# JacobYuan7/DIN-Group-Activity-Recognition-Benchmark

Hardware: AMD Instinct MI355X
Metric: clips/sec (fwd+bwd), Volleyball DIN stage-2, BxTx12 actors (higher is better)
Workload: dtype bf16; 1 GPU; Volleyball stage-2 DIN, inv3, T=3, ST_kernel=(3,3), N=12, 720x1280, bf16; global_batch=32, clips_per_gpu=32, frames=3, parallelism=dp1, includes=fwd + cross-entropy + bwd + fused Adam (lr 0), launch_mode=eager launches, bn_mode=running statistics (set_bn_eval)

## Files before the change

### din-group-activity-recognition-benchmark_amd/_lib.py

```python
from __future__ import annotations

import ctypes as C
import os
import re
import subprocess
from typing import Dict, List

_HERE = os.path.dirname(os.path.abspath(__file__))
LIB_PATH = os.environ.get("DIN_LIB_PATH") or os.path.join(_HERE, "libdin_hip.so")
CSRC_DIR = os.path.join(_HERE, "csrc")
HEADER_PATH = os.path.join(os.path.dirname(_HERE), "include", "din_hip.h")

DIN_F32, DIN_BF16 = 0, 1
ABI_VERSION = 9
CONV_BIAS, CONV_RELU, CONV_ACCUM, CONV_MASK = 1, 2, 4, 8


class DinError(RuntimeError):
    pass


class ConvDesc(C.Structure):
    _fields_ = [(n, C.c_int32) for n in (
        "nb", "h", "w", "cin", "oh", "ow", "cout", "kh", "kw", "sh", "sw", "ph", "pw", "dh", "dw",
# ... 23 lines not shown
    _fields_ = [("desc", ConvDesc), ("in_", C.c_void_p), ("dout", C.c_void_p), ("dw", C.c_void_p), ("dbias", C.c_void_p), ("scale", C.c_void_p),
                ("w", C.c_void_p), ("wdot", C.c_void_p), ("accumulate", C.c_int32), ("reserved", C.c_int32)]


_P, _I, _L, _F, _U64 = C.c_void_p, C.c_int, C.c_int64, C.c_float, C.c_uint64
_CD, _PD = C.POINTER(ConvDesc), C.POINTER(PoolDesc)

SIGNATURES: Dict[str, tuple] = {
    "din_abi_version": (_I, []),
    "din_last_error_string": (C.c_char_p, []),
    "din_set_option": (_I, [C.c_char_p, C.c_char_p]),
    "din_get_option": (_I, [C.c_char_p, C.c_char_p, _I]),
    "din_build_arch": (C.c_char_p, []),
    "din_prep_images_f32": (_I, [_P, _P, _L, _P]),
    "din_prep_images_nhwc": (_I, [_P, _I, _P, _I, _I, _I, _I, _I, _P]),
    "din_conv_packed_elems": (_L, [_CD, _I]),
    "din_conv_pack_weights": (_I, [_CD, _P, _P, _P, _I, _P]),
    "din_conv_pack_desc": (_I, [_CD, _P, _P, _P, _I, C.POINTER(PackDesc)]),
    "din_conv_pack_multi": (_I, [_P, _P, _P, _I, _I, _P]),
    "din_conv_kernel_tile": (_I, [_CD, _I, C.POINTER(C.c_int32), C.POINTER(C.c_int32)]),
    "din_conv_kernel_variant": (_I, [_CD, _I, C.POINTER(C.c_int32)]),
    "din_conv_workspace_bytes": (_L, [_CD, _I]),
    "din_conv_accepts_u8": (_I, [_P]),
    "din_conv_fwd": (_I, [_CD, _P, _P, _P, _P, _I, _P, _L, _P]),
    "din_conv_fwd2": (_I, [_CD, _P, _P, _P, _P, _P, _I, _I, _I, _I, _I, _P, _L, _P]),
    "din_conv_dgrad": (_I, [_CD, _P, _P, _P, _P, _I, _I, _I, _P, _L, _P]),
    "din_conv1x1_dgrad_multi": (_I, [_I, C.POINTER(ConvSrc), _I, _I, _I, _I, _I, _I, _I, _P, _P, _I, _I, _I, _P]),
    "din_conv_dgrad_x_fused": (_I, [_CD]),
    "din_conv_dgrad_x": (_I, [_CD, _P, _P, _P, _P, _I, _I, _I, C.POINTER(ConvSrc), _P, _L, _P]),
    "din_conv1x1_wgrad_multi_workspace": (_L, [_I, C.POINTER(ConvWSrc), _I, _L, _I]),
    "din_conv1x1_wgrad_multi": (_I, [_I, C.POINTER(ConvWSrc), _I, _L, _I, _I, _I, _P, _I, _P, _L, _P]),
    "din_conv_wgrad_group_key": (_I, [_CD]),
    "din_conv_wgrad_group_workspace": (_L, [_I, C.POINTER(ConvWgradItem)]),
    "din_conv_wgrad_group": (_I, [_I, C.POINTER(ConvWgradItem), _P, _L, _P]),
    "din_conv_wgrad": (_I, [_CD, _P, _P, _P, _P, _P, _P, _P, _I, _P, _L, _P]),
    "din_colsum": (_I, [_P, _I, _L, _I, _I, _I, _P, _P]),
    "din_bn_fold": (_I, [_P, _P, _P, _P, _F, _P, _P, _I, _P]),
    "din_bn_fold_bwd": (_I, [_P, _P, _P, _P, _F, _P, _P, _I, _P]),
    "din_bn_fold_multi": (_I, [_P, _P, _I, _I, _F, _P, _P, _P]),
    "din_bn_fold_bwd_multi": (_I, [_P, _P, _I, _I, _F, _P, _P, _P, _P, _P]),
    "din_bn_stats": (_I, [_P, _I, _L, _I, _I, _I, _P, _P, _P]),
    "din_bn_parts": (_I, [_L]),
    "din_bn_workspace": (_L, [_L, _I]),
    "din_bn_reduce": (_I, [_P, _I, _I, _P]),
    "din_bn_finalize": (_I, [_P, _I, _L, _I, _P, _P, _F, _F, _P, _P, _P, _P, _P, _P, _P, _P]),
    "din_bn_apply": (_I, [_P, _I, _L, _I, _I, _I, _P, _P, _I, _P, _I, _I, _P]),
# ... 114 lines not shown
```

### din-group-activity-recognition-benchmark_amd/csrc/conv_igemm.hip

```cpp
#include "din_common.h"
#include "conv_wgrad.h"
#include "conv_gather.h"
#include <atomic>
#include <unordered_map>
#include <mutex>
#include <stdlib.h>

typedef float f32x4 __attribute__((ext_vector_type(4)));
typedef __bf16 bf16x8 __attribute__((ext_vector_type(8)));
typedef uint32_t u32x4 __attribute__((ext_vector_type(4)));
typedef uint32_t u32x2 __attribute__((ext_vector_type(2)));

using din_wgrad::WgradK;
using din_wgrad::lds_dma16;
using din_gather::ConvK;
using din_gather::out_pixel;
using din_gather::staged_tile_store;

namespace {

#ifndef DIN_GATHER_PRIO
#define DIN_GATHER_PRIO 0
#endif
#ifndef DIN_GATHER_ILV
#define DIN_GATHER_ILV 1
#endif
constexpr int BM = 128;
constexpr int KC = 8;
constexpr int NTHREADS = 256;

__device__ __forceinline__ int lds_slot(int row, int chunk) { return row * KC + (chunk ^ ((row >> 1) & 7)); }

template <typename T> struct Mma;
template <> struct Mma<float> {
    __device__ static void run(const u32x4& a, const u32x4& b, f32x4& c) {
#pragma unroll
        for (int j = 0; j < 4; ++j)
            c = __builtin_amdgcn_mfma_f32_16x16x4f32(__uint_as_float(a[j]), __uint_as_float(b[j]), c, 0, 0, 0);
    }
};
// ... 576 lines not shown
        const int px_l = wm * (BM / WM) + (lane & 15);
#pragma unroll
        for (int i = 0; i < TI; ++i) {
            f32x4 bv = {0.f, 0.f, 0.f, 0.f};
            const int co = co_tile * BN + co_l + i * 16;
            const bool cooked = p.craw <= 0 || co < p.craw;
            if ((p.flags & DIN_CONV_BIAS) && co < p.Cout && cooked) bv = *reinterpret_cast<const f32x4*>(p.bias + co);
#pragma unroll
            for (int j = 0; j < TJ; ++j) {
                f32x4 v = acc[i][j] + bv;
                if ((p.flags & DIN_CONV_RELU) && cooked) {
#pragma unroll
                    for (int e = 0; e < 4; ++e) v[e] = fmaxf(v[e], 0.f);
                }
                unsigned char* dst = smem_raw + (px_l + j * 16) * CPITCH + (co_l + i * 16) * (int)sizeof(T);
                if constexpr (sizeof(T) == 4) *reinterpret_cast<f32x4*>(dst) = v;
                else *reinterpret_cast<u32x2*>(dst) = u32x2{pack_bf16x2(v[0], v[1]), pack_bf16x2(v[2], v[3])};
            }
        }
    }
    staged_tile_store<T, BM, BN, NT>(p, smem_raw, tid, co_tile, m_first);
#endif
}

__device__ __forceinline__ float prep_u8(uint32_t v) {
    float y = __fdiv_rn((float)v, 255.0f);
    y = __fsub_rn(y, 0.5f);
    return __fmul_rn(y, 2.0f);
}
__device__ __forceinline__ void u8_lut_init(bf16_t* lut, int tid) {
    lut[tid] = (bf16_t)(pack_bf16x2(prep_u8((uint32_t)tid), 0.f) & 0xffffu);
}
template <int V> struct IcTag { static constexpr int value = V; };
template <int NTR>
struct U8Halo {
    uint32_t r[NTR], g[NTR], b[NTR];
    uint32_t valid;
    template <int NSLOT>
    __device__ __forceinline__ void load(const unsigned char* __restrict__ img, int n, int H, int W, int gy0, int gx0, int wid,
                                         const short (&hyv)[NTR], const short (&hxv)[NTR], const int (&inside)[NTR]) {
        const int64_t plane = (int64_t)H * W;
        const unsigned char* base = img + (int64_t)n * 3 * plane;
        valid = 0u;
#pragma unroll
        for (int i = 0; i < NTR; ++i) {
            const int gy = gy0 + hyv[i], gx = gx0 + hxv[i];
            const bool ok = wid + 4 * i < NSLOT && inside[i] >= 0 && gy >= 0 && gy < H && gx >= 0 && gx < W;
            const unsigned char* q = base + (int64_t)min(max(gy, 0), H - 1) * W + min(max(gx, 0), W - 1);
            asm volatile("global_load_ubyte %0, %1, off" : "=&v"(r[i]) : "v"(q) : "memory");
            asm volatile("global_load_ubyte %0, %1, off" : "=&v"(g[i]) : "v"(q + plane) : "memory");
            asm volatile("global_load_ubyte %0, %1, off" : "=&v"(b[i]) : "v"(q + 2 * plane) : "memory");
            valid |= (ok ? 1u : 0u) << i;
        }
    }
    __device__ __forceinline__ void landed() {
#pragma unroll
        for (int i = 0; i < NTR; ++i) { asm volatile("" : "+v"(r[i])); asm volatile("" : "+v"(g[i])); asm volatile("" : "+v"(b[i])); }
    }
    template <int NSLOT>
    __device__ __forceinline__ void store(unsigned char* lds_buf, const bf16_t* lut, int wid, int lane) const {
#pragma unroll
        for (int i = 0; i < NTR; ++i) {
            if (wid + 4 * i < NSLOT) {
                u32x4 v = {0u, 0u, 0u, 0u};
                if ((valid >> i) & 1u) {
                    v[0] = (uint32_t)lut[r[i]] | ((uint32_t)lut[g[i]] << 16);
                    v[1] = (uint32_t)lut[b[i]];
                }
                *reinterpret_cast<u32x4*>(lds_buf + ((wid + 4 * i) * 64 + lane) * 16) = v;
            }
        }
    }
};

template <int CPP, int BN, int NBUF, int KH, int KW, int ST, bool U8 = false, int NW = 4, bool EPI = false>
__global__ __launch_bounds__(64 * NW, NW == 8 ? 1 : 2) void conv_small_kernel(ConvK p) {
    constexpr int NTHREADS = 64 * NW;
    static_assert(!U8 || NW == 4, "the uint8 halo loader is written for four waves");
    static_assert(!U8 || (CPP == 1 && NBUF == 2), "uint8 frames feed the image layer only");
#if defined(__HIP_DEVICE_COMPILE__)
    typedef bf16_t T;
    constexpr int TH = 8, TW = 32, NPX = TH * TW;
    constexpr int TI = BN / 16, TJ = 16 / NW, NTAPS = KH * KW;
    constexpr int SL = CPP >= 4 ? CPP / 4 : 1, NSL = CPP >= 4 ? NTAPS * SL : (NTAPS + 3) / 4;
    constexpr int CPITCH = BN * 2 + 16;
    constexpr int HWW = (TW - 1) * ST + KW, HWH = (TH - 1) * ST + KH, HPX = HWW * HWH, HC = HPX * CPP;
    constexpr int WBYTES = NSL * BN * 4 * 16;
    constexpr int HBYTES = (HC * 16 + 1023) / 1024 * 1024;
    constexpr int NSLOT = HBYTES / 1024, NTR = (NSLOT + NW - 1) / NW;
    constexpr int NPASS = HBYTES / CPITCH >= NPX ? 1 : 2;
    static_assert(HBYTES / CPITCH >= NPX / NPASS, "staging does not fit the halo buffer");
    constexpr int JN = TJ / NPASS;
    constexpr int CPR = BN / 8;
    constexpr int NST = (NPX / NPASS) * CPR / NTHREADS * NPASS;
    static_assert((NPX / NPASS) * CPR % NTHREADS == 0, "store loop must be uniform");
    constexpr unsigned OOB = 0x80000000u;
// ... 2989 lines not shown
```

### din-group-activity-recognition-benchmark_amd/nhwc.py

```python
from __future__ import annotations

import ctypes as C
from dataclasses import dataclass, field
from typing import Dict, List, Optional, Sequence, Tuple

import torch

from . import _lib as L


def _ptr(t: Optional[torch.Tensor]):
    return C.c_void_p(t.data_ptr()) if t is not None else None


def _stream():
    return C.c_void_p(torch.cuda.current_stream().cuda_stream)


def torch_dtype(dt: int):
    return torch.float32 if dt == L.DIN_F32 else torch.bfloat16


def din_dtype(t: torch.Tensor) -> int:
    if t.dtype == torch.float32:
# ... 19 lines not shown


def _timed(kind, d, name=""):
    return LAUNCH_TIMER(kind, d, name) if LAUNCH_TIMER is not None else _contextlib.nullcontext()


GRAD_HOOK = None
GRAD_TAP = None
GRAD_BUFFER = None
GRAD_ASSIGN = None


def _dw_buffer(w: torch.Tensor) -> torch.Tensor:
    if GRAD_BUFFER is not None:
        buf = GRAD_BUFFER(w)
        if buf is not None:
            return buf
    return torch.empty_like(w)
FUSE_1X1_DGRAD = None
FUSE_FWD_SIBLINGS = None
FUSE_WGRAD_SIBLINGS = None
FUSE_WGRAD_1X1 = None
FUSE_DGRAD_X = None
GROUP_WGRAD = None
GROUP_WGRAD_MAX = 12
GROUP_WGRAD_MB = 768
_SWITCHES = {"FUSE_1X1_DGRAD": ("DIN_FUSE_1X1", True), "FUSE_FWD_SIBLINGS": ("DIN_FUSE_FWD", True), "FUSE_WGRAD_SIBLINGS": ("DIN_FUSE_WGRAD", True),
             "FUSE_WGRAD_1X1": ("DIN_FUSE_WGRAD_1X1", True), "FUSE_DGRAD_X": ("DIN_FUSE_DGRAD_X", True), "GROUP_WGRAD": ("DIN_GROUP_WGRAD", True), "WGRAD_SIDE_STREAM": ("DIN_WGRAD_STREAM", False)}


def switch(attr: str) -> bool:
    v = globals()[attr]
    if v is not None:
        return bool(v)
    name, default = _SWITCHES[attr]
    return L.host_flag(name, default)



_WS: Dict[Tuple[int, str], torch.Tensor] = {}


_SIDE: Dict[int, "torch.cuda.Stream"] = {}
WGRAD_SIDE_STREAM = None


def side_stream(device) -> "torch.cuda.Stream":
    key = device.index if device.index is not None else torch.cuda.current_device()
    if key not in _SIDE:
        _SIDE[key] = torch.cuda.Stream(device=device)
    return _SIDE[key]
# ... 270 lines not shown
            op = g.ops[oi]
            d = _conv_desc(g, op, 1, dt, op.src.c)
            w, scale_ptr = src_of[oi]
            pd = L.PackDesc()
            L.check(lib.din_conv_pack_desc(C.byref(d), _ptr(w), scale_ptr, _ptr(fused), 0, C.byref(pd)), "conv_pack_desc(fused)")
            pd.out = fused.data_ptr() + row0 * pd.kelems * esz
            pd.rows_pad = pd.rows
            li = len(descs)
            descs.append(pd)
            nchunk = (pd.rows * pd.kelems + PACK_CHUNK - 1) // PACK_CHUNK
            layer_of += [li] * nchunk
            chunk_index += list(range(nchunk))
            row0 += op.dst.c
    raw = (L.PackDesc * len(descs))(*descs)
    host = torch.frombuffer(bytearray(bytes(raw)), dtype=torch.uint8).clone()
    pc.table = host.to(dev)
    pc.layer_of = torch.tensor(layer_of, dtype=torch.int32).to(dev)
    pc.chunk_index = torch.tensor(chunk_index, dtype=torch.int32).to(dev)
    pc.nblocks = len(layer_of)
    g._pack_cache = pc
    return pc


BN_MOMENTUM = 0.1


def _bn_train_forward(lib, raw: torch.Tensor, dt: int, rows: int, cout: int, gamma, beta, mean, var, relu: bool, dst: torch.Tensor,
                      ldd: int, coffd: int, st):
    dev = raw.device
    ws = torch.empty(lib.din_bn_workspace(rows, cout) // 8, dtype=torch.float64, device=dev)
    ab = torch.empty(4 * cout, dtype=torch.float32, device=dev)
    a, b, bmean, rstd = ab[:cout], ab[cout:2 * cout], ab[2 * cout:3 * cout], ab[3 * cout:]
    L.check(lib.din_bn_stats(_ptr(raw), dt, rows, cout, cout, 0, None, _ptr(ws), st), "bn_stats")
    L.check(lib.din_bn_finalize(_ptr(ws), lib.din_bn_parts(rows), rows, cout, _ptr(gamma), _ptr(beta), BN_EPS, BN_MOMENTUM, _ptr(mean), _ptr(var),
                                _ptr(a), _ptr(b), _ptr(bmean), _ptr(rstd), None, st), "bn_finalize")
    L.check(lib.din_bn_apply(_ptr(raw), dt, rows, cout, cout, 0, _ptr(a), _ptr(b), int(relu), _ptr(dst), ldd, coffd, st), "bn_apply")
    return bmean, rstd


def graph_forward(g: Graph, image_buf: torch.Tensor, params: Sequence[torch.Tensor], dt: int, save_for_backward: bool = True,
                  bn_train: bool = False):
    lib = L.load()
    nb = image_buf.shape[0]
    dev = image_buf.device
    tdt = torch_dtype(dt)
    bufs: List[Optional[torch.Tensor]] = [None] * len(g.tensors)
    bufs[g.input_tid] = image_buf
    it = iter(params)
    aux = []
    st = _stream()
    bn = _bn_tables(g, params, dev)
    pc = _pack_cache(g, params, dt, dev, save_for_backward, bn)
    bn_train = bool(bn_train) and bn is not None
    if bn_train:
        bn_scale, bn_shift = pc.bn_scale, pc.bn_shift
        bn_scale.fill_(1.0)
    elif bn is not None:
        bn_scale, bn_shift = pc.bn_scale, pc.bn_shift
        L.check(lib.din_bn_fold_multi(_ptr(bn.ptrs), _ptr(bn.offs), bn.n, bn.total, BN_EPS, _ptr(bn_scale), _ptr(bn_shift), st), "bn_fold_multi")
    L.check(lib.din_conv_pack_multi(_ptr(pc.table), _ptr(pc.layer_of), _ptr(pc.chunk_index), pc.nblocks, PACK_CHUNK, st), "conv_pack_multi")
    bn_i = 0
    group_of = {grp[0]: grp for grp in g.fwd_groups} if (switch("FUSE_FWD_SIBLINGS") and not bn_train) else {}
    fused_done = set()
    for oi, op in enumerate(g.ops):
        td = g.tensors[op.dst.tid]
        if bufs[op.dst.tid] is None:
            bufs[op.dst.tid] = torch.empty((nb, td.h, td.w, td.c), dtype=tdt, device=dev)
        src, dst = bufs[op.src.tid], bufs[op.dst.tid]
        if op.kind == "conv":
            cin = g.cin_image if op.src.tid == g.input_tid else op.src.c
            d = _conv_desc(g, op, nb, dt, cin)
            if op.src.tid == g.input_tid and src.dtype == torch.uint8:
                d.in_u8, d.ldi, d.cioff = 1, 8, 0
            w = next(it)
            scale = shift = None
            if op.bn:
                gamma, beta, mean, var = next(it), next(it), next(it), next(it)
                o0, o1 = bn.off_list[bn_i], bn.off_list[bn_i + 1]
                bn_i += 1
                scale, shift = bn_scale[o0:o1], bn_shift[o0:o1]
                bias = shift
            else:
                bias = next(it) if op.bias else None
            if op.bn and bn_train:
                dR = _conv_desc(g, op, nb, dt, cin)
                dR.in_u8, dR.ldi, dR.cioff = d.in_u8, d.ldi, d.cioff
                dR.ldo, dR.cooff = op.dst.c, 0
                raw = torch.empty((nb, g.tensors[op.src.tid].h if op.pooled is not None else td.h,
                                   g.tensors[op.src.tid].w if op.pooled is not None else td.w, op.dst.c), dtype=tdt, device=dev)
                if op.pooled is not None:
                    dR.oh, dR.ow = raw.shape[1], raw.shape[2]
                ws, wsb = workspace(lib.din_conv_workspace_bytes(C.byref(dR), 0), dev)
                with _timed("fwd", dR, op.name):
                    L.check(lib.din_conv_fwd(C.byref(dR), _ptr(src), _ptr(pc.wpk[oi]), None, _ptr(raw), 0, _ptr(ws), wsb, st), "conv_fwd " + op.name)
                if op.pooled is not None:
                    _, pd = _pooled_descs(g, op, nb, dt)
                    pd.ldo, pd.cooff = op.dst.c, 0
                    pooled_raw = torch.empty((nb, td.h, td.w, op.dst.c), dtype=tdt, device=dev)
                    L.check(lib.din_avgpool_fwd(C.byref(pd), _ptr(raw), _ptr(pooled_raw), None, 0, st), "avgpool_fwd(raw)")
                    raw = pooled_raw
                bmean, rstd = _bn_train_forward(lib, raw, dt, nb * td.h * td.w, op.dst.c, gamma, beta, mean, var, op.relu, dst, td.c,
                                                op.dst.coff, st)
                aux.append((None, raw if save_for_backward else None, bmean, rstd))
                continue
            if oi in fused_done:
                if op.pooled is not None:
                    _, pd = _pooled_descs(g, op, nb, dt)
                    pd.ldi, pd.cioff = g.tensors[op.mid.tid].c, op.mid.coff
                    L.check(lib.din_avgpool_fwd(C.byref(pd), _ptr(bufs[op.mid.tid]), _ptr(dst), _ptr(bias),
                                                L.CONV_BIAS | (L.CONV_RELU if op.relu else 0), st), "avgpool_fwd(epilogue)")
                aux.append((scale,))
                continue
            if oi in group_of and op.bn:
                grp = group_of[oi]
                rest = [g.ops[i] for i in grp[1:]]
                ctot = op.dst.c + sum(o.dst.c for o in rest)
                craw = ctot - sum(o.dst.c for o in rest if o.pooled is not None)
                dF = _conv_desc(g, op, nb, dt, cin)
                dF.cout = ctot
                v2 = group_view(rest[0])
                t2 = v2.tid
                td2 = g.tensors[t2]
                if lib.din_conv_workspace_bytes(C.byref(dF), 0) == 0 and bn.off_list[bn_i - 1 + len(grp)] - o0 == ctot:
                    if bufs[t2] is None:
                        bufs[t2] = torch.empty((nb, td2.h, td2.w, td2.c), dtype=tdt, device=dev)
                    flags = L.CONV_BIAS | (L.CONV_RELU if op.relu else 0)
# ... 581 lines not shown
```

### din-group-activity-recognition-benchmark_amd/profiling.py

```python
from __future__ import annotations

import ctypes as C
import os

import torch

from . import _lib as L
from . import nhwc

PROFILE = None
PROFILE_ONLY = None
HBM = None


def _conv_flops(d) -> float:
    over = getattr(d, "flops_override", None)
    return float(over) if over else 2.0 * d.nb * d.oh * d.ow * d.cout * d.cin * d.kh * d.kw


def _esz(dt: int) -> int:
    return 4 if dt == L.DIN_F32 else 2


def _stem_bytes(kind: str, d) -> float:
    e = _esz(d.dtype)
    x = d.nb * d.h * d.w * (3 if d.in_u8 else d.cin * e)
    y = d.nb * d.oh * d.ow * d.cout * e
    if kind == "fwd":
        return float(x + y)
    if kind == "dgrad":
        return float(y + 2 * x)
    return float(x + y)


def _pool_bytes(name: str, args) -> float:
    d = args[0]._obj
    e = _esz(d.dtype)
    big, small = d.nb * d.h * d.w * d.c, d.nb * d.oh * d.ow * d.c
    if name == "din_maxpool_fwd":
        return float(e * (big + small) + (small if args[3] else 0))
    return float(e * (small + big) + (small if args[2] else e * big) + (e * big if args[6] else 0))


def _roi_bytes(name: str, args) -> float:
    if name == "din_roi_align_fwd":
        _fm, dt, nb, hf, wf, c, _ldf, _gh, _gw, _b, _i, m, k = args[:13]
        return float(nb * hf * wf * c * _esz(dt) + m * c * k * k * 4)
    if name == "din_roi_crop_grad_transpose":
# ... 47 lines not shown
            setattr(lib, name, fn)
        self.records, HBM = HBM, None
        return False

    def summary(self, event_overhead_ms: float = 0.0, peak_gbs: float = 8000.0):
        out = {}
        for group, _name, nbytes, e0, e1 in self.records:
            rec = out.setdefault(group, [0.0, 0.0, 0])
            rec[0] += nbytes
            rec[1] += max(e0.elapsed_time(e1) - event_overhead_ms, 1e-4) * 1e-3
            rec[2] += 1
        return {g: {"bound": "hbm", "achieved": round(v[0] / v[1] / 1e9, 1), "peak": peak_gbs, "unit": "GB/s",
                    "frac": round(v[0] / v[1] / 1e9 / peak_gbs, 4), "launches": v[2], "time_ms": round(v[1] * 1e3, 3),
                    "algorithmic_bytes": round(v[0])} for g, v in out.items()}


class LaunchTimer:
    def __init__(self, kind, d, name=""):
        self.kind, self.d, self.name = kind, d, name
        self.rec = False

    def _variant(self) -> str:
        d = self.d
        bm, bn = C.c_int32(0), C.c_int32(0)
        which = {"fwd": 0, "dgrad": 1, "wgrad": 2}[self.kind]
        L.load().din_conv_kernel_tile(C.byref(d), which, C.byref(bm), C.byref(bn))
        tn = "unsigned short" if d.dtype == L.DIN_BF16 else "float"
        if self.kind == "wgrad":
            if self.name.startswith("1x1multi:"):
                return f"conv_wgrad_1x1_multi_kernel<{d.cin // 8}>"
            if self.name.startswith("group:"):
                return f"conv_wgrad_pipe_group_kernel<{bm.value}, {bn.value - 2000}, {'true' if d.ow >= 32 else 'false'}, 8>"
            if bm.value == 3:
                return f"conv_wgrad_halo_kernel<..., {bn.value}, ...>"
            if bm.value == 0:
                return f"conv_wgrad_small_kernel<..., {bn.value}, ...>"
            if bn.value >= 2000:
                waves = int(L.get_option("DIN_WGRAD_PIPE_WAVES") or "16")
                wn = 8 if waves == 16 else (2 if waves == 4 and bm.value <= 192 else 4)
                return f"conv_wgrad_pipe_kernel<{bm.value}, {bn.value - 2000}, {'true' if d.ow >= 32 else 'false'}, {wn}>"
            if bn.value >= 1000:
                return f"conv_wgrad_ring_kernel<{bm.value}, {bn.value - 1000}>"
            return f"conv_wgrad_bf16_kernel<{bm.value}>" if d.dtype == L.DIN_BF16 else "conv_wgrad_f32_kernel"
        if bm.value == 4 and not (self.kind == "dgrad" and "+" in self.name):
            return f"conv1x1_stream_kernel<{bn.value}>"
        if bm.value == 5:
# ... 16 lines not shown
        if BM == 256:
            geo = "4, 1, 4, 4" if BN == 64 else ("2, 2, 8, 2" if BN in (96, 160) else "4, 2, 8, 2")
        elif multi:
            geo = "4, 2, 8, 2" if (BN % 64 == 0 and d.dtype == L.DIN_BF16) else "2, 2, 8, 2"
        else:
            geo = "4, 2, 8, 2" if fl.value & 2 else "2, 2, 8, 2"
        return (f"conv_gather_fast_kernel<{tn}, {BM}, {BN}, {geo}, {'true' if multi else 'false'}, "
                f"{'true' if fl.value & 1 else 'false'}, false, {'true' if fl.value & 4 else 'false'}>")

    def __enter__(self):
        if PROFILE is not None:
            self.variant = self._variant()
            if PROFILE_ONLY is None or self.variant == PROFILE_ONLY:
                self.rec = True
                self.e0 = torch.cuda.Event(enable_timing=True)
                self.e1 = torch.cuda.Event(enable_timing=True)
                self.e0.record(torch.cuda.current_stream())
        return self

    def __exit__(self, *exc):
        if self.rec:
            self.e1.record(torch.cuda.current_stream())
            PROFILE.append((self.kind, self.variant, _conv_flops(self.d), int(self.d.dtype), self.e0, self.e1, self.name))
            if HBM is not None and self.variant.startswith(("conv_small_kernel", "conv_wgrad_small_kernel")):
                HBM.append(("stem (Conv2d_1a-2b halo kernels)", self.variant, _stem_bytes(self.kind, self.d), self.e0, self.e1))
        return False




def install() -> None:
    nhwc.LAUNCH_TIMER = LaunchTimer
    nhwc.TIMING_ACTIVE = lambda: PROFILE is not None


def uninstall() -> None:
    nhwc.LAUNCH_TIMER = None
    nhwc.TIMING_ACTIVE = lambda: False
```

### include/din_hip.h

```cpp
#ifndef DIN_HIP_H
#define DIN_HIP_H

#include <stddef.h>
#include <stdint.h>

#ifdef __cplusplus
extern "C" {
#endif

#define DIN_ABI_VERSION 9

enum { DIN_F32 = 0, DIN_BF16 = 1 };

enum {
    DIN_OK = 0,
    DIN_E_ARG = -1,
    DIN_E_LAUNCH = -2,
    DIN_E_WORKSPACE = -3,
    DIN_E_UNSUPPORTED = -4
};

int din_abi_version(void);
const char* din_last_error_string(void);
const char* din_build_arch(void);
// ... 19 lines not shown
    DIN_CONV_ACCUM = 4,
    DIN_CONV_MASK = 8
};

int64_t din_conv_packed_elems(const din_conv_desc* d, int transposed);
int din_conv_pack_weights(const din_conv_desc* d, const float* w, const float* scale, void* wpk,
                          int transposed, void* stream);
typedef struct din_pack_desc {
    uint64_t w, scale, out;
    int32_t cout, cin, kh, kw;
    int32_t rows, rows_pad, inner, inner_pad, kelems, transposed, dtype;
    int32_t reserved;
} din_pack_desc;
int din_conv_pack_desc(const din_conv_desc* d, const float* w, const float* scale, void* wpk, int transposed, din_pack_desc* out);
int din_conv_pack_multi(const din_pack_desc* table, const int32_t* layer_of, const int32_t* chunk_index, int nblocks,
                        int chunk_elems, void* stream);
int din_conv_fwd2(const din_conv_desc* d, const void* in, const void* wpk, const float* bias, void* out, void* out2, int ldo2, int cooff2,
                  int csplit, int craw, int flags, void* workspace, int64_t workspace_bytes, void* stream);
int din_conv_kernel_tile(const din_conv_desc* d, int which, int32_t* bm, int32_t* bn);
int din_conv_kernel_variant(const din_conv_desc* d, int which, int32_t* flags);
int64_t din_conv_workspace_bytes(const din_conv_desc* d, int which );

int din_conv_accepts_u8(const din_conv_desc* d);

int din_conv_fwd(const din_conv_desc* d, const void* in, const void* wpk, const float* bias, void* out,
                 int flags, void* workspace, int64_t workspace_bytes, void* stream);
int din_conv_dgrad(const din_conv_desc* d, const void* dout, const void* wpk_t, void* din,
                   const void* mask, int ldm, int moff, int flags,
                   void* workspace, int64_t workspace_bytes, void* stream);
typedef struct din_conv_src {
    const void* dout;
    const void* wpk_t;
    int32_t cout, ldo, cooff;
} din_conv_src;
int din_conv1x1_dgrad_multi(int nsrc, const din_conv_src* srcs, int dtype, int nb, int h, int w, int cin, int ldi,
                            int cioff, void* din, const void* mask, int ldm, int moff, int flags, void* stream);
int din_conv_dgrad_x(const din_conv_desc* d, const void* dout, const void* wpk_t, void* din, const void* mask, int ldm, int moff, int flags,
                     const din_conv_src* x, void* workspace, int64_t workspace_bytes, void* stream);
int din_conv_dgrad_x_fused(const din_conv_desc* d);
int din_conv_wgrad(const din_conv_desc* d, const void* in, const void* dout, float* dw, float* dbias,
                   const float* scale, const float* w, float* wdot, int accumulate,
                   void* workspace, int64_t workspace_bytes, void* stream);

typedef struct din_conv_wsrc {
    const void* dout;
    float* dw;
// ... 144 lines not shown
```

Baseline: 651.2 clips/sec.

## Fuse uint8 stem conv 1a and conv 2a into one halo-tiled kernel

Adds a fused forward kernel that reads uint8 frames, computes the stride-2 3x3 first conv into an LDS halo tile, and feeds it straight into the 3x3 32->32 second conv. The intermediate activation is written to HBM only when it is needed for backward. The goal is to cut the HBM round trip and one launch on the two largest-resolution stem layers. In exchange the kernel recomputes the halo pixels of the first conv at tile borders and requires a persistent tile loop with register and LDS prefetch. It only applies when BN is in eval mode and the input is uint8.

```diff
diff --git a/din-group-activity-recognition-benchmark_amd/_lib.py b/din-group-activity-recognition-benchmark_amd/_lib.py
--- a/din-group-activity-recognition-benchmark_amd/_lib.py
+++ b/din-group-activity-recognition-benchmark_amd/_lib.py
@@ -69,6 +69,8 @@
     "din_conv_kernel_variant": (_I, [_CD, _I, C.POINTER(C.c_int32)]),
     "din_conv_workspace_bytes": (_L, [_CD, _I]),
     "din_conv_accepts_u8": (_I, [_P]),
+    "din_conv_stem_fused": (_I, [_CD, _CD]),
+    "din_conv_stem_fwd": (_I, [_CD, _CD, _P, _P, _P, _P, _P, _P, _P, _I, _P]),
     "din_conv_fwd": (_I, [_CD, _P, _P, _P, _P, _I, _P, _L, _P]),
     "din_conv_fwd2": (_I, [_CD, _P, _P, _P, _P, _P, _I, _I, _I, _I, _I, _P, _L, _P]),
     "din_conv_dgrad": (_I, [_CD, _P, _P, _P, _P, _I, _I, _I, _P, _L, _P]),
diff --git a/din-group-activity-recognition-benchmark_amd/csrc/conv_igemm.hip b/din-group-activity-recognition-benchmark_amd/csrc/conv_igemm.hip
--- a/din-group-activity-recognition-benchmark_amd/csrc/conv_igemm.hip
+++ b/din-group-activity-recognition-benchmark_amd/csrc/conv_igemm.hip
@@ -1,6 +1,7 @@
 #include "din_common.h"
 #include "conv_wgrad.h"
 #include "conv_gather.h"
+#include "conv_u8.h"
 #include <atomic>
 #include <unordered_map>
 #include <mutex>
@@ -16,6 +17,9 @@
 using din_gather::ConvK;
 using din_gather::out_pixel;
 using din_gather::staged_tile_store;
+using din_u8::U8Halo;
+using din_u8::IcTag;
+using din_u8::u8_lut_init;
 
 namespace {
 
@@ -638,56 +642,6 @@
     staged_tile_store<T, BM, BN, NT>(p, smem_raw, tid, co_tile, m_first);
 #endif
 }
-
-__device__ __forceinline__ float prep_u8(uint32_t v) {
-    float y = __fdiv_rn((float)v, 255.0f);
-    y = __fsub_rn(y, 0.5f);
-    return __fmul_rn(y, 2.0f);
-}
-__device__ __forceinline__ void u8_lut_init(bf16_t* lut, int tid) {
-    lut[tid] = (bf16_t)(pack_bf16x2(prep_u8((uint32_t)tid), 0.f) & 0xffffu);
-}
-template <int V> struct IcTag { static constexpr int value = V; };
-template <int NTR>
-struct U8Halo {
-    uint32_t r[NTR], g[NTR], b[NTR];
-    uint32_t valid;
-    template <int NSLOT>
-    __device__ __forceinline__ void load(const unsigned char* __restrict__ img, int n, int H, int W, int gy0, int gx0, int wid,
-                                         const short (&hyv)[NTR], const short (&hxv)[NTR], const int (&inside)[NTR]) {
-        const int64_t plane = (int64_t)H * W;
-        const unsigned char* base = img + (int64_t)n * 3 * plane;
-        valid = 0u;
-#pragma unroll
-        for (int i = 0; i < NTR; ++i) {
-            const int gy = gy0 + hyv[i], gx = gx0 + hxv[i];
-            const bool ok = wid + 4 * i < NSLOT && inside[i] >= 0 && gy >= 0 && gy < H && gx >= 0 && gx < W;
-            const unsigned char* q = base + (int64_t)min(max(gy, 0), H - 1) * W + min(max(gx, 0), W - 1);
-            asm volatile("global_load_ubyte %0, %1, off" : "=&v"(r[i]) : "v"(q) : "memory");
-            asm volatile("global_load_ubyte %0, %1, off" : "=&v"(g[i]) : "v"(q + plane) : "memory");
-            asm volatile("global_load_ubyte %0, %1, off" : "=&v"(b[i]) : "v"(q + 2 * plane) : "memory");
-            valid |= (ok ? 1u : 0u) << i;
-        }
-    }
-    __device__ __forceinline__ void landed() {
-#pragma unroll
-        for (int i = 0; i < NTR; ++i) { asm volatile("" : "+v"(r[i])); asm volatile("" : "+v"(g[i])); asm volatile("" : "+v"(b[i])); }
-    }
-    template <int NSLOT>
-    __device__ __forceinline__ void store(unsigned char* lds_buf, const bf16_t* lut, int wid, int lane) const {
-#pragma unroll
-        for (int i = 0; i < NTR; ++i) {
-            if (wid + 4 * i < NSLOT) {
-                u32x4 v = {0u, 0u, 0u, 0u};
-                if ((valid >> i) & 1u) {
-                    v[0] = (uint32_t)lut[r[i]] | ((uint32_t)lut[g[i]] << 16);
-                    v[1] = (uint32_t)lut[b[i]];
-                }
-                *reinterpret_cast<u32x4*>(lds_buf + ((wid + 4 * i) * 64 + lane) * 16) = v;
-            }
-        }
-    }
-};
 
 template <int CPP, int BN, int NBUF, int KH, int KW, int ST, bool U8 = false, int NW = 4, bool EPI = false>
 __global__ __launch_bounds__(64 * NW, NW == 8 ? 1 : 2) void conv_small_kernel(ConvK p) {
diff --git a/din-group-activity-recognition-benchmark_amd/csrc/conv_stem_fused.hip b/din-group-activity-recognition-benchmark_amd/csrc/conv_stem_fused.hip
--- /dev/null
+++ b/din-group-activity-recognition-benchmark_amd/csrc/conv_stem_fused.hip
@@ -0,0 +1,275 @@
+#include "din_common.h"
+#include "conv_gather.h"
+#include "conv_u8.h"
+#include <stdlib.h>
+
+typedef float f32x4 __attribute__((ext_vector_type(4)));
+typedef __bf16 bf16x8 __attribute__((ext_vector_type(8)));
+typedef uint32_t u32x4 __attribute__((ext_vector_type(4)));
+typedef uint32_t u32x2 __attribute__((ext_vector_type(2)));
+
+namespace {
+
+struct StemK {
+    const unsigned char* u8; const void* w1; const float* b1; void* a1; const void* w2; const float* b2; void* out;
+    int NB, H, W;
+    int OH1, OW1, ldo1, cooff1;
+    int OH, OW, ldo, cooff;
+    int wld1, wld2, flags2;
+};
+
+constexpr int SF_TH = 8, SF_TW = 32, SF_C = 32;
+constexpr int SF_AH = SF_TH + 2, SF_AW = SF_TW + 2, SF_APX = SF_AH * SF_AW;
+constexpr int SF_ASEG = (SF_APX + 15) / 16;
+constexpr int SF_BH = 2 * (SF_AH - 1) + 3, SF_BW = 2 * (SF_AW - 1) + 3, SF_BPX = SF_BH * SF_BW;
+constexpr int SF_WBYTES = 9 * SF_C * 4 * 16;
+constexpr int SF_ABYTES = (SF_APX * 64 + 1023) / 1024 * 1024;
+constexpr int SF_BBYTES = (SF_BPX * 16 + 1023) / 1024 * 1024;
+constexpr int SF_LDS = SF_WBYTES + SF_ABYTES + SF_BBYTES + 512;
+constexpr int SF_CPITCH = SF_C * 2 + 16;
+static_assert(SF_ABYTES >= SF_TH * SF_TW * SF_CPITCH, "the A2 staging tile must fit the consumed A1 halo buffer");
+static_assert(SF_LDS <= 65536, "two workgroups per CU");
+
+__device__ __forceinline__ void mma_bf16(const u32x4& a, const u32x4& b, f32x4& c) {
+    c = __builtin_amdgcn_mfma_f32_16x16x32_bf16(__builtin_bit_cast(bf16x8, a), __builtin_bit_cast(bf16x8, b), c, 0, 0, 0);
+}
+
+__global__ __launch_bounds__(256, 2) void conv_stem_fused_kernel(StemK p) {
+#if defined(__HIP_DEVICE_COMPILE__)
+    constexpr int NW = 4, NTHREADS = 256;
+    constexpr int NSLOT = SF_BBYTES / 1024, NTR = (NSLOT + NW - 1) / NW;
+    constexpr int NSEG = (SF_ASEG + NW - 1) / NW;
+    constexpr int NA1 = (SF_APX * 4 + NTHREADS - 1) / NTHREADS;
+    constexpr int TI = 2, TJ = 4, NIT = SF_TH * SF_TW * 4 / NTHREADS;
+    constexpr unsigned OOB = 0x80000000u;
+    extern __shared__ __attribute__((aligned(16))) unsigned char smem_raw[];
+    const int tid = threadIdx.x, lane = tid & 63, wid = tid >> 6;
+    const int frow = lane & 15, g4 = lane >> 4;
+    u32x4* Wl = reinterpret_cast<u32x4*>(smem_raw);
+    unsigned char* Ab = smem_raw + SF_WBYTES;
+    unsigned char* Bb = Ab + SF_ABYTES;
+    bf16_t* lut = reinterpret_cast<bf16_t*>(Bb + SF_BBYTES);
+    auto swz = [](int row) { return (row >> 1) & 3; };
+
+    din_u8::u8_lut_init(lut, tid);
+    {
+        const u32x4* __restrict__ wp = reinterpret_cast<const u32x4*>(p.w2);
+        for (int id = tid; id < 9 * SF_C * 4; id += NTHREADS) {
+            const int row = id >> 2, slot = id & 3;
+            const int tap = row / SF_C, co = row - tap * SF_C;
+            Wl[id] = wp[(int64_t)co * p.wld2 + tap * 4 + (slot ^ swz(co))];
+        }
+    }
+    u32x4 wf1[3][TI];
+    f32x4 bias1[TI], bias2[TI];
+    {
+        const u32x4* __restrict__ wp = reinterpret_cast<const u32x4*>(p.w1);
+#pragma unroll
+        for (int sl = 0; sl < 3; ++sl)
+#pragma unroll
+            for (int i = 0; i < TI; ++i) wf1[sl][i] = wp[(int64_t)(i * 16 + frow) * p.wld1 + sl * 4 + g4];
+#pragma unroll
+        for (int i = 0; i < TI; ++i) {
+            const int co = i * 16 + g4 * 4;
+            bias1[i] = *reinterpret_cast<const f32x4*>(p.b1 + co);
+            bias2[i] = f32x4{0.f, 0.f, 0.f, 0.f};
+            if (p.flags2 & DIN_CONV_BIAS) bias2[i] = *reinterpret_cast<const f32x4*>(p.b2 + co);
+        }
+#pragma unroll
+        for (int sl = 0; sl < 3; ++sl)
+#pragma unroll
+            for (int i = 0; i < TI; ++i) asm volatile("" : "+v"(wf1[sl][i]));
+#pragma unroll
+        for (int i = 0; i < TI; ++i) { asm volatile("" : "+v"(bias1[i])); asm volatile("" : "+v"(bias2[i])); }
+    }
+    short hyv[NTR], hxv[NTR];
+    int inside[NTR];
+#pragma unroll
+    for (int i = 0; i < NTR; ++i) {
+        const int id = (wid + NW * i) * 64 + lane;
+        const int hy = id / SF_BW;
+        hyv[i] = (short)hy; hxv[i] = (short)(id - hy * SF_BW);
+        inside[i] = id < SF_BPX ? 0 : -1;
+    }
+    const int tiles_x = (p.OW + SF_TW - 1) / SF_TW, tiles_y = (p.OH + SF_TH - 1) / SF_TH;
+    const int tiles_img = tiles_x * tiles_y, ntiles = tiles_img * p.NB;
+    const long long oimg_bytes = (long long)p.OH * p.OW * p.ldo * 2ll, aimg_bytes = (long long)p.OH1 * p.OW1 * p.ldo1 * 2ll;
+    const bool relu2 = (p.flags2 & DIN_CONV_RELU) != 0;
+    const bool keep_a1 = p.a1 != nullptr;
+
+    din_u8::U8Halo<NTR> u8h;
+    auto u8_load = [&](int t) {
+        const int n = t / tiles_img;
+        const int tr = t - n * tiles_img;
+        const int ty = tr / tiles_x, tx = tr - ty * tiles_x;
+        u8h.template load<NSLOT>(p.u8, n, p.H, p.W, ty * SF_TH * 2, tx * SF_TW * 2, wid, hyv, hxv, inside);
+    };
+    int tile = xcd_remap((int)blockIdx.x, (int)gridDim.x);
+    __syncthreads();
+    if (tile < ntiles) {
+        u8_load(tile);
+        asm volatile("s_waitcnt vmcnt(0)" ::: "memory"); u8h.landed();
+        u8h.template store<NSLOT>(Bb, lut, wid, lane);
+    }
+    for (; tile < ntiles; tile += gridDim.x) {
+        __syncthreads();
+        const bool have_next = tile + (int)gridDim.x < ntiles;
+        if (have_next) u8_load(tile + gridDim.x);
+        const int n = tile / tiles_img;
+        const int trm = tile - n * tiles_img;
+        const int ty = trm / tiles_x, tx = trm - ty * tiles_x;
+        const int ay0 = ty * SF_TH, ax0 = tx * SF_TW;
+        {
+            const u32x4* Bl = reinterpret_cast<const u32x4*>(Bb);
+#pragma unroll
+            for (int j = 0; j < NSEG; ++j) {
+                const int hpr = (wid + NW * j) * 16 + frow;
+                const int hp = min(hpr, SF_APX - 1);
+                const int hy = hp / SF_AW, hx = hp - hy * SF_AW;
+                f32x4 acc[TI] = {f32x4{0.f, 0.f, 0.f, 0.f}, f32x4{0.f, 0.f, 0.f, 0.f}};
+#pragma unroll
+                for (int sl = 0; sl < 3; ++sl) {
+                    const int tap = min(sl * 4 + g4, 8);
+                    const int r = tap / 3, s2 = tap - r * 3;
+                    const u32x4 xf = Bl[(hy * 2 + r) * SF_BW + hx * 2 + s2];
+#pragma unroll
+                    for (int i = 0; i < TI; ++i) mma_bf16(wf1[sl][i], xf, acc[i]);
+                }
+                const bool live = ay0 + hy < p.OH1 && ax0 + hx < p.OW1;
+                if (hpr < SF_APX) {
+#pragma unroll
+                    for (int i = 0; i < TI; ++i) {
+                        f32x4 v = acc[i] + bias1[i];
+#pragma unroll
+                        for (int e = 0; e < 4; ++e) v[e] = fmaxf(v[e], 0.f);
+                        u32x2 o = {pack_bf16x2(v[0], v[1]), pack_bf16x2(v[2], v[3])};
+                        if (!live) o = u32x2{0u, 0u};
+                        const int chunk = i * 2 + (g4 >> 1);
+                        *reinterpret_cast<u32x2*>(Ab + (hp * 4 + (chunk ^ swz(hp))) * 16 + (g4 & 1) * 8) = o;
+                    }
+                }
+            }
+        }
+        __syncthreads();
+        const u32x4* Al = reinterpret_cast<const u32x4*>(Ab);
+        if (keep_a1) {
+            __amdgpu_buffer_rsrc_t rsA = __builtin_amdgcn_make_buffer_rsrc(reinterpret_cast<char*>(p.a1) + (long long)n * aimg_bytes, 0, (int)aimg_bytes, 0x00020000);
+            const int own_h = ty == tiles_y - 1 ? SF_AH : SF_TH, own_w = tx == tiles_x - 1 ? SF_AW : SF_TW;
+#pragma unroll
+            for (int it = 0; it < NA1; ++it) {
+                const int id = min(it * NTHREADS + tid, SF_APX * 4 - 1);
+                const int hp = id >> 2, cc = (id & 3) ^ swz(hp);
+                const int hy = hp / SF_AW, hx = hp - hy * SF_AW;
+                const bool ok = it * NTHREADS + tid < SF_APX * 4 && hy < own_h && hx < own_w && ay0 + hy < p.OH1 && ax0 + hx < p.OW1;
+                const u32x4 v = Al[id];
+                __builtin_amdgcn_raw_buffer_store_b128(v, rsA, ok ? (((ay0 + hy) * p.OW1 + ax0 + hx) * p.ldo1 + p.cooff1 + cc * 8) * 2 : (int)OOB, 0, 0);
+            }
+        }
+        f32x4 acc[TI][TJ];
+#pragma unroll
+        for (int i = 0; i < TI; ++i)
+#pragma unroll
+            for (int j = 0; j < TJ; ++j) acc[i][j] = f32x4{0.f, 0.f, 0.f, 0.f};
+#pragma unroll
+        for (int tap = 0; tap < 9; ++tap) {
+            const int dy = tap / 3, dx = tap - dy * 3;
+            u32x4 wf[TI], xf[TJ];
+#pragma unroll
+            for (int i = 0; i < TI; ++i) {
+                const int co = i * 16 + frow;
+                wf[i] = Wl[(tap * SF_C + co) * 4 + (g4 ^ swz(co))];
+            }
+#pragma unroll
+            for (int j = 0; j < TJ; ++j) {
+                const int q = wid * TJ + j;
+                const int hp = ((q >> 1) + dy) * SF_AW + (q & 1) * 16 + frow + dx;
+                xf[j] = Al[hp * 4 + (g4 ^ swz(hp))];
+            }
+#pragma unroll
+            for (int i = 0; i < TI; ++i)
+#pragma unroll
+                for (int j = 0; j < TJ; ++j) mma_bf16(wf[i], xf[j], acc[i][j]);
+        }
+        if (have_next) {
+            if (keep_a1) asm volatile("s_waitcnt vmcnt(%0)" :: "n"(NA1) : "memory");
+            else asm volatile("s_waitcnt vmcnt(0)" ::: "memory");
+            u8h.landed();
+            u8h.template store<NSLOT>(Bb, lut, wid, lane);
+        }
+        __syncthreads();
+#pragma unroll
+        for (int i = 0; i < TI; ++i) {
+            const int co = i * 16 + g4 * 4;
+#pragma unroll
+            for (int j = 0; j < TJ; ++j) {
+                f32x4 v = acc[i][j] + bias2[i];
+                if (relu2) {
+#pragma unroll
+                    for (int e = 0; e < 4; ++e) v[e] = fmaxf(v[e], 0.f);
+                }
+                const int srow = (wid * TJ + j) * 16 + frow;
+                *reinterpret_cast<u32x2*>(Ab + srow * SF_CPITCH + co * 2) = u32x2{pack_bf16x2(v[0], v[1]), pack_bf16x2(v[2], v[3])};
+            }
+        }
+        __syncthreads();
+        __amdgpu_buffer_rsrc_t rsO = __builtin_amdgcn_make_buffer_rsrc(reinterpret_cast<char*>(p.out) + (long long)n * oimg_bytes, 0, (int)oimg_bytes, 0x00020000);
+#pragma unroll
+        for (int it = 0; it < NIT; ++it) {
+            const int idx = it * NTHREADS + tid;
+            const int srow = idx >> 2, c = idx & 3;
+            const int w_ = srow / (TJ * 16), rem = srow - w_ * (TJ * 16);
+            const int q = w_ * TJ + rem / 16;
+            const int gy = ty * SF_TH + (q >> 1), gx = tx * SF_TW + (q & 1) * 16 + (rem & 15);
+            const bool ok = gy < p.OH && gx < p.OW;
+            const u32x4 v = *reinterpret_cast<const u32x4*>(Ab + srow * SF_CPITCH + c * 16);
+            __builtin_amdgcn_raw_buffer_store_b128(v, rsO, ok ? ((gy * p.OW + gx) * p.ldo + p.cooff + c * 8) * 2 : (int)OOB, 0, 0);
+        }
+    }
+#endif
+}
+
+bool stem_pair_ok(const din_conv_desc* d1, const din_conv_desc* d2) {
+    if (!d1 || !d2 || !din_conv_accepts_u8(d1) || d1->cout != SF_C || d1->ph != 0 || d1->pw != 0) return false;
+    if (d2->dtype != DIN_BF16 || d2->in_u8 || d2->kh != 3 || d2->kw != 3 || d2->sh != 1 || d2->sw != 1 || d2->ph != 0 || d2->pw != 0 ||
+        d2->dh != 1 || d2->dw != 1 || d2->cin != SF_C || d2->cout != SF_C) return false;
+    if (d2->nb != d1->nb || d2->h != d1->oh || d2->w != d1->ow || d2->oh != d2->h - 2 || d2->ow != d2->w - 2 || d2->oh <= 0 || d2->ow <= 0) return false;
+    if (d1->oh != (d1->h - 3) / 2 + 1 || d1->ow != (d1->w - 3) / 2 + 1) return false;
+    if (d2->ldo % 8 != 0 || d2->cooff % 8 != 0 || d2->ldo < d2->cooff + SF_C || d1->ldo < d1->cooff + SF_C) return false;
+    if ((long long)d2->oh * d2->ow * d2->ldo * 2 >= 0x7fffffffll || (int64_t)d2->nb * d2->oh * d2->ow < 256 * 1024) return false;
+    return true;
+}
+
+}
+
+extern "C" {
+
+int din_conv_stem_fused(const din_conv_desc* d1, const din_conv_desc* d2) {
+    return stem_pair_ok(d1, d2) ? 1 : 0;
+}
+
+int din_conv_stem_fwd(const din_conv_desc* d1, const din_conv_desc* d2, const void* frames, const void* wpk1, const float* bias1, void* a1,
+                      const void* wpk2, const float* bias2, void* out, int flags2, void* stream) {
+    DIN_REQUIRE(d1 && d2, "conv_stem_fwd: null descriptor");
+    DIN_REQUIRE(d1->in_u8 == 1, "conv_stem_fwd: the image layer must read uint8 frames (in_u8)");
+    DIN_REQUIRE(stem_pair_ok(d1, d2), "conv_stem_fwd: not a uint8 image layer (3x3 / stride 2, 3 -> 32) followed by a 3x3 / stride 1 / pad 0, "
+                "32 -> 32 bf16 conv over >= 256 Ki pixels (see din_conv_stem_fused)");
+    DIN_REQUIRE(frames && wpk1 && bias1 && wpk2 && out, "conv_stem_fwd: null pointer");
+    DIN_REQUIRE(!(flags2 & ~(DIN_CONV_BIAS | DIN_CONV_RELU)), "conv_stem_fwd: only BIAS / RELU apply to the second conv");
+    DIN_REQUIRE(!(flags2 & DIN_CONV_BIAS) || bias2, "conv_stem_fwd: BIAS flag without bias");
+    StemK k{};
+    k.u8 = reinterpret_cast<const unsigned char*>(frames); k.w1 = wpk1; k.b1 = bias1; k.a1 = a1; k.w2 = wpk2; k.b2 = bias2; k.out = out;
+    k.NB = d1->nb; k.H = d1->h; k.W = d1->w;
+    k.OH1 = d1->oh; k.OW1 = d1->ow; k.ldo1 = d1->ldo; k.cooff1 = d1->cooff;
+    k.OH = d2->oh; k.OW = d2->ow; k.ldo = d2->ldo; k.cooff = d2->cooff;
+    k.wld1 = (9 * 1 + 7) / 8 * 8; k.wld2 = (9 * 4 + 7) / 8 * 8;
+    k.flags2 = flags2;
+    const char* gv = DIN_OPT("DIN_STEM_FUSE_GRID");
+    const int tiles = ((k.OH + SF_TH - 1) / SF_TH) * ((k.OW + SF_TW - 1) / SF_TW) * k.NB;
+    int grid = gv && atoi(gv) > 0 ? atoi(gv) : 512;
+    if (grid > tiles) grid = tiles;
+    hipLaunchKernelGGL(conv_stem_fused_kernel, dim3(grid), dim3(256), SF_LDS, as_stream(stream), k);
+    DIN_CHECK_LAUNCH("conv_stem_fwd");
+    return DIN_OK;
+}
+
+}
diff --git a/din-group-activity-recognition-benchmark_amd/csrc/conv_u8.h b/din-group-activity-recognition-benchmark_amd/csrc/conv_u8.h
--- /dev/null
+++ b/din-group-activity-recognition-benchmark_amd/csrc/conv_u8.h
@@ -0,0 +1,57 @@
+#pragma once
+#include "din_common.h"
+#include "conv_gather.h"
+
+namespace din_u8 {
+
+__device__ __forceinline__ float prep_u8(uint32_t v) {
+    float y = __fdiv_rn((float)v, 255.0f);
+    y = __fsub_rn(y, 0.5f);
+    return __fmul_rn(y, 2.0f);
+}
+__device__ __forceinline__ void u8_lut_init(bf16_t* lut, int tid) {
+    lut[tid] = (bf16_t)(pack_bf16x2(prep_u8((uint32_t)tid), 0.f) & 0xffffu);
+}
+template <int V> struct IcTag { static constexpr int value = V; };
+template <int NTR>
+struct U8Halo {
+    uint32_t r[NTR], g[NTR], b[NTR];
+    uint32_t valid;
+    template <int NSLOT>
+    __device__ __forceinline__ void load(const unsigned char* __restrict__ img, int n, int H, int W, int gy0, int gx0, int wid,
+                                         const short (&hyv)[NTR], const short (&hxv)[NTR], const int (&inside)[NTR]) {
+        const int64_t plane = (int64_t)H * W;
+        const unsigned char* base = img + (int64_t)n * 3 * plane;
+        valid = 0u;
+#pragma unroll
+        for (int i = 0; i < NTR; ++i) {
+            const int gy = gy0 + hyv[i], gx = gx0 + hxv[i];
+            const bool ok = wid + 4 * i < NSLOT && inside[i] >= 0 && gy >= 0 && gy < H && gx >= 0 && gx < W;
+            const unsigned char* q = base + (int64_t)min(max(gy, 0), H - 1) * W + min(max(gx, 0), W - 1);
+            asm volatile("global_load_ubyte %0, %1, off" : "=&v"(r[i]) : "v"(q) : "memory");
+            asm volatile("global_load_ubyte %0, %1, off" : "=&v"(g[i]) : "v"(q + plane) : "memory");
+            asm volatile("global_load_ubyte %0, %1, off" : "=&v"(b[i]) : "v"(q + 2 * plane) : "memory");
+            valid |= (ok ? 1u : 0u) << i;
+        }
+    }
+    __device__ __forceinline__ void landed() {
+#pragma unroll
+        for (int i = 0; i < NTR; ++i) { asm volatile("" : "+v"(r[i])); asm volatile("" : "+v"(g[i])); asm volatile("" : "+v"(b[i])); }
+    }
+    template <int NSLOT>
+    __device__ __forceinline__ void store(unsigned char* lds_buf, const bf16_t* lut, int wid, int lane) const {
+#pragma unroll
+        for (int i = 0; i < NTR; ++i) {
+            if (wid + 4 * i < NSLOT) {
+                din_u32x4 v = {0u, 0u, 0u, 0u};
+                if ((valid >> i) & 1u) {
+                    v[0] = (uint32_t)lut[r[i]] | ((uint32_t)lut[g[i]] << 16);
+                    v[1] = (uint32_t)lut[b[i]];
+                }
+                *reinterpret_cast<din_u32x4*>(lds_buf + ((wid + 4 * i) * 64 + lane) * 16) = v;
+            }
+        }
+    }
+};
+
+}
diff --git a/din-group-activity-recognition-benchmark_amd/nhwc.py b/din-group-activity-recognition-benchmark_amd/nhwc.py
--- a/din-group-activity-recognition-benchmark_amd/nhwc.py
+++ b/din-group-activity-recognition-benchmark_amd/nhwc.py
@@ -65,11 +65,12 @@
 FUSE_WGRAD_SIBLINGS = None
 FUSE_WGRAD_1X1 = None
 FUSE_DGRAD_X = None
+STEM_FUSE = None
 GROUP_WGRAD = None
 GROUP_WGRAD_MAX = 12
 GROUP_WGRAD_MB = 768
 _SWITCHES = {"FUSE_1X1_DGRAD": ("DIN_FUSE_1X1", True), "FUSE_FWD_SIBLINGS": ("DIN_FUSE_FWD", True), "FUSE_WGRAD_SIBLINGS": ("DIN_FUSE_WGRAD", True),
-             "FUSE_WGRAD_1X1": ("DIN_FUSE_WGRAD_1X1", True), "FUSE_DGRAD_X": ("DIN_FUSE_DGRAD_X", True), "GROUP_WGRAD": ("DIN_GROUP_WGRAD", True), "WGRAD_SIDE_STREAM": ("DIN_WGRAD_STREAM", False)}
+             "FUSE_WGRAD_1X1": ("DIN_FUSE_WGRAD_1X1", True), "FUSE_DGRAD_X": ("DIN_FUSE_DGRAD_X", True), "GROUP_WGRAD": ("DIN_GROUP_WGRAD", True), "STEM_FUSE": ("DIN_STEM_FUSE", True), "WGRAD_SIDE_STREAM": ("DIN_WGRAD_STREAM", False)}
 
 
 def switch(attr: str) -> bool:
@@ -386,6 +387,24 @@
     return pc
 
 
+def _stem_fuse_descs(g: Graph, nb: int, dt: int):
+    if not switch("STEM_FUSE") or len(g.ops) < 2:
+        return None
+    a, b = g.ops[0], g.ops[1]
+    if a.kind != "conv" or b.kind != "conv" or a.src.tid != g.input_tid or not (a.bn and a.relu and b.bn) or a.pooled or b.pooled:
+        return None
+    ta = g.tensors[a.dst.tid]
+    if (a.dst.coff, a.dst.c) != (0, ta.c) or (b.src.tid, b.src.coff, b.src.c) != (a.dst.tid, 0, ta.c):
+        return None
+    if a.dst.tid in g.output_tids or any(o.src.tid == a.dst.tid or o.dst.tid == a.dst.tid for o in g.ops[2:]):
+        return None
+    if any(i in grp for grp in g.fwd_groups for i in (0, 1)):
+        return None
+    d1, d2 = _conv_desc(g, a, nb, dt, g.cin_image), _conv_desc(g, b, nb, dt, b.src.c)
+    d1.in_u8, d1.ldi, d1.cioff = 1, 8, 0
+    return (d1, d2) if L.load().din_conv_stem_fused(C.byref(d1), C.byref(d2)) else None
+
+
 BN_MOMENTUM = 0.1
 
 
@@ -426,9 +445,13 @@
     bn_i = 0
     group_of = {grp[0]: grp for grp in g.fwd_groups} if (switch("FUSE_FWD_SIBLINGS") and not bn_train) else {}
     fused_done = set()
+    stem = _stem_fuse_descs(g, nb, dt) if (image_buf.dtype == torch.uint8 and not bn_train) else None
+    stem_bias = None
     for oi, op in enumerate(g.ops):
         td = g.tensors[op.dst.tid]
-        if bufs[op.dst.tid] is None:
+        if stem is not None and oi == 0 and not save_for_backward:
+            pass
+        elif bufs[op.dst.tid] is None:
             bufs[op.dst.tid] = torch.empty((nb, td.h, td.w, td.c), dtype=tdt, device=dev)
         src, dst = bufs[op.src.tid], bufs[op.dst.tid]
         if op.kind == "conv":
@@ -466,6 +489,19 @@
                 bmean, rstd = _bn_train_forward(lib, raw, dt, nb * td.h * td.w, op.dst.c, gamma, beta, mean, var, op.relu, dst, td.c,
                                                 op.dst.coff, st)
                 aux.append((None, raw if save_for_backward else None, bmean, rstd))
+                continue
+            if stem is not None and oi == 0:
+                stem_bias = bias
+                aux.append((scale,))
+                continue
+            if stem is not None and oi == 1:
+                d1, d2 = stem
+                d2.stem_fused = (d1, bufs[op.src.tid] is not None)
+                flags = L.CONV_BIAS | (L.CONV_RELU if op.relu else 0)
+                with _timed("fwd", d2, g.ops[0].name + "+" + op.name):
+                    L.check(lib.din_conv_stem_fwd(C.byref(d1), C.byref(d2), _ptr(image_buf), _ptr(pc.wpk[0]), _ptr(stem_bias), _ptr(src),
+                                                  _ptr(pc.wpk[oi]), _ptr(bias), _ptr(dst), flags, st), "conv_stem_fwd " + op.name)
+                aux.append((scale,))
                 continue
             if oi in fused_done:
                 if op.pooled is not None:
diff --git a/din-group-activity-recognition-benchmark_amd/profiling.py b/din-group-activity-recognition-benchmark_amd/profiling.py
--- a/din-group-activity-recognition-benchmark_amd/profiling.py
+++ b/din-group-activity-recognition-benchmark_amd/profiling.py
@@ -15,7 +15,9 @@
 
 def _conv_flops(d) -> float:
     over = getattr(d, "flops_override", None)
-    return float(over) if over else 2.0 * d.nb * d.oh * d.ow * d.cout * d.cin * d.kh * d.kw
+    own = 2.0 * d.nb * d.oh * d.ow * d.cout * d.cin * d.kh * d.kw
+    fused = getattr(d, "stem_fused", None)
+    return float(over) if over else own + (_conv_flops(fused[0]) if fused else 0.0)
 
 
 def _esz(dt: int) -> int:
@@ -24,6 +26,10 @@
 
 def _stem_bytes(kind: str, d) -> float:
     e = _esz(d.dtype)
+    fused = getattr(d, "stem_fused", None)
+    if fused:
+        d1, kept = fused
+        return float(d1.nb * d1.h * d1.w * 3 + (d1.nb * d1.oh * d1.ow * d1.cout * e if kept else 0) + d.nb * d.oh * d.ow * d.cout * e)
     x = d.nb * d.h * d.w * (3 if d.in_u8 else d.cin * e)
     y = d.nb * d.oh * d.ow * d.cout * e
     if kind == "fwd":
@@ -117,6 +123,8 @@
 
     def _variant(self) -> str:
         d = self.d
+        if getattr(d, "stem_fused", None):
+            return "conv_stem_fused_kernel"
         bm, bn = C.c_int32(0), C.c_int32(0)
         which = {"fwd": 0, "dgrad": 1, "wgrad": 2}[self.kind]
         L.load().din_conv_kernel_tile(C.byref(d), which, C.byref(bm), C.byref(bn))
@@ -179,7 +187,7 @@
         if self.rec:
             self.e1.record(torch.cuda.current_stream())
             PROFILE.append((self.kind, self.variant, _conv_flops(self.d), int(self.d.dtype), self.e0, self.e1, self.name))
-            if HBM is not None and self.variant.startswith(("conv_small_kernel", "conv_wgrad_small_kernel")):
+            if HBM is not None and self.variant.startswith(("conv_small_kernel", "conv_wgrad_small_kernel", "conv_stem_fused_kernel")):
                 HBM.append(("stem (Conv2d_1a-2b halo kernels)", self.variant, _stem_bytes(self.kind, self.d), self.e0, self.e1))
         return False
 
diff --git a/include/din_hip.h b/include/din_hip.h
--- a/include/din_hip.h
+++ b/include/din_hip.h
@@ -65,6 +65,10 @@
 int64_t din_conv_workspace_bytes(const din_conv_desc* d, int which );
 
 int din_conv_accepts_u8(const din_conv_desc* d);
+
+int din_conv_stem_fused(const din_conv_desc* d1, const din_conv_desc* d2);
+int din_conv_stem_fwd(const din_conv_desc* d1, const din_conv_desc* d2, const void* frames, const void* wpk1, const float* bias1, void* a1,
+                      const void* wpk2, const float* bias2, void* out, int flags2, void* stream);
 
 int din_conv_fwd(const din_conv_desc* d, const void* in, const void* wpk, const float* bias, void* out,
                  int flags, void* workspace, int64_t workspace_bytes, void* stream);
```

Measured after the change: 651.1 clips/sec (median of 2 runs). Within noise of the previous version (-0.0%).
